# ETM-Code/eirgrid

Hardware: AMD Instinct MI355X
Metric: 26-year episodes/sec (higher is better)
Workload: dtype f64

## Files before the change

### eirgrid_amd/csrc/eg_api.cpp

```cpp
#include <algorithm>
#include <cstdlib>
#include <cstring>

#include "eg_device_tables.h"
#include "eg_host.h"
#include "eg_policy_internal.h"

namespace eg {
namespace {
thread_local std::string g_error;
}
void set_error(const std::string& s) { g_error = s; }
}

using namespace eg;

void eg_host_tables::index() {
  auto F = [&](const char* n, const std::vector<double>& v) { f64[n] = {v.data(), (int64_t)v.size()}; };
  auto I = [&](const char* n, const std::vector<int32_t>& v) { i32[n] = {v.data(), (int64_t)v.size()}; };
  F("usage", H.usage); F("population", H.population); F("pre_co2", H.pre_co2); F("pre_tg", H.pre_tg); F("pre_ig", H.pre_ig);
  F("pre_sg", H.pre_sg); F("pre_optot", H.pre_optot); F("te", H.te); F("coastf", H.coastf); F("dr", H.dr); F("m03", H.m03);
  F("t12", H.t12); F("cc", H.cc); F("out_mw", H.out_mw); F("co2_t", H.co2_t); F("offv", H.offv); F("offc", H.offc);
  F("inflation", H.inflation); F("carbon_price", H.carbon_price);
  f64["size_factor"] = {&H.size_factor, 1};
  I("pre_opcnt", H.pre_opcnt); I("cls", H.cls); I("rclass", H.rclass); I("marine", H.marine); I("reach", H.reach);
  I("existing_online", H.existing_online);
}

namespace {
struct Options {
  bool helper_off = false, helper_all = false;
  bool heavy_slots_auto = true; uint32_t heavy_slots_wanted = 4096;
  uint32_t heavy_slots_max = 0;
  bool side_stream_plain = false;
  bool replay_hoist = false;
  int coop_force = 0;
  bool solo_on = true;
  uint32_t solo_tiles = 1u;
};
Options read_options() {
  Options o;
  if (const char* hv = std::getenv("EIRGRID_HELPER_WAVES")) { o.helper_off = std::string(hv) == "0"; o.helper_all = std::string(hv) == "all"; }
  if (const char* hs = std::getenv("EIRGRID_HEAVY_SLOTS")) { o.heavy_slots_wanted = (uint32_t)std::strtoul(hs, nullptr, 10); o.heavy_slots_auto = false; }
  o.heavy_slots_max = uint32_t((size_t(64) << 30) / (size_t(kRadiusClasses) * 2624 * sizeof(double)));
  if (const char* hg = std::getenv("EIRGRID_HEAVY_POOL_GB"))
    o.heavy_slots_max = uint32_t(std::min(double((1u << 20) - 1u), std::max(0.0, std::atof(hg)) * double(size_t(1) << 30) / double(size_t(kRadiusClasses) * 2624 * sizeof(double))));
  if (o.heavy_slots_max > (1u << 20) - 1u) o.heavy_slots_max = (1u << 20) - 1u;
  if (o.heavy_slots_wanted > o.heavy_slots_max) o.heavy_slots_wanted = o.heavy_slots_max;
  if (const char* sp = std::getenv("EIRGRID_SIDE_STREAM")) o.side_stream_plain = std::string(sp) == "plain";
  if (const char* rh = std::getenv("EIRGRID_REPLAY_HOIST")) o.replay_hoist = rh[0] == '1';
  if (const char* cf = std::getenv("EIRGRID_COOP_FORCE")) o.coop_force = std::atoi(cf);
  if (const char* so = std::getenv("EIRGRID_REPLAY_SOLO")) o.solo_on = so[0] != '0';
  if (const char* st = std::getenv("EIRGRID_SOLO_TILES")) o.solo_tiles = st[0] != '0' ? 1u : 0u;
  return o;
}

int collect_timing(eg_ctx* c, int count = -1) {
  if (count < 0 || count > c->ring_pending) count = c->ring_pending;
  for (; count > 0; --count) {
    const int i = (c->ring_head - c->ring_pending + 2 * eg_ctx::kTimingRing) % eg_ctx::kTimingRing;
    const bool heavy = c->ev_used[i] & 1, lean = c->ev_used[i] & 2;
    float best = 0.f, sum = 0.f;
    for (int a = 0; a < 2; ++a)
      for (int b = 0; b < 2; ++b) {
        if (!(a ? lean : heavy) || !(b ? lean : heavy)) continue;
        EG_HIP(hipEventSynchronize(c->ev[i][2 * b + 1]));
        float ms = 0.f;
        EG_HIP(hipEventElapsedTime(&ms, c->ev[i][2 * a], c->ev[i][2 * b + 1]));
        if (a == b) sum += ms;
        if (ms > best) best = ms;
      }
    c->total_ms += double(best); c->grids_ms += double(sum); c->n_launches += 1; c->ring_pending -= 1;
  }
  return EG_OK;
}
}
static bool env_starts(const char* name, char ch) { const char* e = std::getenv(name); return e && e[0] == ch; }
bool eg::stats_replicas_off() { static const bool off = env_starts("EIRGRID_STATS_REPLICAS", '0'); return off; }
bool eg::fetch_full() { static const bool full = env_starts("EIRGRID_FETCH_FULL", '1'); return full; }

int eg::ensure_outputs(eg_ctx* c, uint32_t n) {
  const size_t bytes = size_t(n) * rec::stride + size_t(n) * sizeof(double);
  if (bytes <= c->d_out.count) return EG_OK;
  c->out = DevOut{};
  EG_HIP(c->d_out.reserve(bytes));
  c->out.base = c->d_out;
// ... 198 lines not shown
  return EG_OK;
}

extern "C" {

const char* eg_last_error(void) { return g_error.c_str(); }

int32_t eg_device_count(void) {
  int n = 0;
  if (hipGetDeviceCount(&n) != hipSuccess) return 0;
  return n;
}

eg_ctx* eg_create(int32_t device_ordinal, const eg_world* world) {
  if (!world || world->n_settlements < 0 || world->n_existing < 0 || world->n_coast < 0) { set_error("eg_create: bad world"); return nullptr; }
  int n = 0;
  if (hipGetDeviceCount(&n) != hipSuccess || n <= 0) { set_error("eg_create: no HIP device (this library has no CPU path)"); return nullptr; }
  if (device_ordinal < 0 || device_ordinal >= n) { set_error("eg_create: device ordinal out of range"); return nullptr; }
  if (hipSetDevice(device_ordinal) != hipSuccess) { set_error("eg_create: hipSetDevice failed"); return nullptr; }
  int cus = 0;
  if (hipDeviceGetAttribute(&cus, hipDeviceAttributeMultiprocessorCount, device_ordinal) != hipSuccess) cus = 0;
  const Options opt = read_options();
  eg_ctx* c = new eg_ctx();
  c->device = device_ordinal;
  c->helper_max_episodes = opt.helper_off ? 0u : opt.helper_all ? 0xFFFFFFFFu : 4u * (uint32_t)(cus > 0 ? cus : 0);
  c->heavy_slots_wanted = opt.heavy_slots_wanted; c->heavy_slots_auto = opt.heavy_slots_auto; c->heavy_slots_max = opt.heavy_slots_max;
  build_tables(*world, c->tables.H);
  c->tables.index();
  std::vector<uint8_t> blob;
  BlobInfo info;
  int rc = build_device_blob(c->tables.H, blob, info);
  if (rc == EG_OK) {
    c->dev.n_variants = info.n_variants; c->dev.size_factor = c->tables.H.size_factor; c->dev.n_existing = world->n_existing;
    c->dev.solo_tiles = opt.solo_tiles;
    if (!info.box_list_fits) c->heavy_slots_wanted = 0;
    c->hoist_supported = info.hoist_supported; c->hoist_on = info.hoist_supported && opt.replay_hoist;
    c->coop_force = opt.coop_force; c->solo_on = opt.solo_on;
    rc = create_device_state(c, blob, opt.side_stream_plain);
  }
  if (rc != EG_OK) { eg_destroy(c); return nullptr; }
  return c;
}

void eg_destroy(eg_ctx* c) {
  if (!c) return;
  (void)hipSetDevice(c->device);
  (void)hipDeviceSynchronize();
  for (int i = 0; i < eg_ctx::kTimingRing; ++i)
    for (int k = 0; k < 4; ++k) if (c->ev[i][k]) (void)hipEventDestroy(c->ev[i][k]);
  if (c->stream_heavy) (void)hipStreamDestroy(c->stream_heavy);
  for (int i = 0; i < eg_ctx::kTimingRing; ++i) { if (c->ev_fork[i]) (void)hipEventDestroy(c->ev_fork[i]); if (c->ev_go[i]) (void)hipEventDestroy(c->ev_go[i]); if (c->ev_join[i]) (void)hipEventDestroy(c->ev_join[i]); }
  delete c;
}

eg_host_tables* eg_host_tables_create(const eg_world* world) {
  if (!world || world->n_settlements < 0 || world->n_existing < 0 || world->n_coast < 0) { set_error("eg_host_tables_create: bad world"); return nullptr; }
  eg_host_tables* h = new eg_host_tables();
  build_tables(*world, h->H);
  h->index();
  return h;
}
void eg_host_tables_free(eg_host_tables* h) { delete h; }
int32_t eg_host_tables_f64(const eg_host_tables* h, const char* name, const double** ptr, int64_t* len) {
  return h ? find_table("eg_host_tables_f64", h->f64, name, ptr, len) : EG_ERR_BAD_ARG;
}
int32_t eg_host_tables_i32(const eg_host_tables* h, const char* name, const int32_t** ptr, int64_t* len) {
  return h ? find_table("eg_host_tables_i32", h->i32, name, ptr, len) : EG_ERR_BAD_ARG;
// ... 240 lines not shown
```

### eirgrid_amd/csrc/eg_internal.h

```cpp
#pragma once
#include <cstddef>
#include <cstdint>
#include <string>
#include <vector>

#include "eirgrid_hip.h"

namespace eg {

constexpr int kYears = EG_YEARS;
constexpr int kTypes = EG_N_TYPES;
constexpr int kCells = EG_CELLS;
constexpr int kGrid = EG_GRID;
constexpr int kRadiusClasses = 6;
constexpr int kMaxReach = 12;
constexpr int kMults = 3;
constexpr int kOffsetTypes = 4;
constexpr int kPsStride = 2624;
constexpr int kDrCompact = 352;
constexpr int kLdsGens = EG_ONCHIP_GENS;
constexpr int kShortReplayMax = 96;
constexpr int kMaxVariants = 12;
constexpr int kTileW = 8;
constexpr int kTileCols = (kGrid + kTileW - 1) / kTileW;
// ... 60 lines not shown
constexpr size_t m03 = a16(dr + 8 * kRadiusClasses * 169);
constexpr size_t t12 = a16(m03 + 8 * kCells);
constexpr size_t offv = a16(t12 + 8 * kYears * kTypes);
constexpr size_t offc = a16(offv + 8 * kYears * kOffsetTypes * kYears);
constexpr size_t cc = a16(offc + 8 * kYears * kOffsetTypes * kMults);
constexpr size_t ps = a16(cc + 8 * size_t(kYears) * kTypes * kYears * kMults * 2);
constexpr size_t hv_box = a16(ps + sizeof(PsRec) * size_t(kYears) * kMaxVariants * kPsStride);
constexpr size_t dr_meta = a16(hv_box + 4 * (1024 + 16));
constexpr size_t dr_compact = a16(dr_meta + 4 * 16);
constexpr size_t pbase = a16(dr_compact + 8 * size_t(kDrCompact));
constexpr size_t pcell = a16(pbase + 8 * size_t(kYears) * kMaxVariants * kPcStride);
constexpr size_t hv_lists = a16(pcell + 4 * size_t(kYears) * kMaxVariants * kPcStride);
constexpr size_t hv_quads = a16(hv_lists + 4 * size_t(64) * 1024);
constexpr size_t te_cell = a16(hv_quads + 4 * 64);
constexpr size_t coastf = a16(te_cell + 8 * size_t(kYears) * kRadiusClasses * kCells);
constexpr size_t cbase = a16(coastf + 8 * size_t(kCells));
constexpr size_t crank = a16(cbase + 8 * size_t(kYears) * kMaxVariants * kCells);
constexpr size_t ucell = a16(crank + 2 * size_t(kYears) * kMaxVariants * kCells);
constexpr size_t umax = a16(ucell + 8 * size_t(kMaxVariants) * kCells);
constexpr size_t rmax = a16(umax + 8 * size_t(kMaxVariants) * 64);
constexpr size_t total = a16(rmax + 8 * size_t(kYears) * kMaxVariants * 64);
}

struct DevTables {
  const uint8_t* base;
  double size_factor;
  int32_t n_existing;
  int32_t n_variants;
  uint32_t heavy_slots, heavy_epoch;
  uint8_t* heavy;
  unsigned* heavy_claim;
  double* heavy_tiles;
  uint32_t solo_tiles;
#define EG_TAB(name, type) EG_HD const type* name() const { return reinterpret_cast<const type*>(base + tab::name); }
  EG_TAB(usage, double) EG_TAB(population, double)
  EG_TAB(pre_co2, double) EG_TAB(pre_tg, double) EG_TAB(pre_ig, double) EG_TAB(pre_sg, double) EG_TAB(pre_optot, double)
  EG_TAB(inflation, double) EG_TAB(carbon_price, double) EG_TAB(out_mw, double) EG_TAB(co2_t, double)
  EG_TAB(pre_opcnt, int32_t) EG_TAB(variant, int32_t) EG_TAB(cls, int32_t) EG_TAB(rclass, int32_t) EG_TAB(marine, int32_t)
  EG_TAB(reach, int32_t)
  EG_TAB(dr, double) EG_TAB(m03, double) EG_TAB(t12, double) EG_TAB(offv, double) EG_TAB(offc, double) EG_TAB(cc, double)
  EG_TAB(ps, PsRec) EG_TAB(pbase, double) EG_TAB(pcell, uint32_t) EG_TAB(hv_lists, uint32_t) EG_TAB(hv_quads, int32_t) EG_TAB(dr_meta, int32_t) EG_TAB(dr_compact, double)
  EG_TAB(te_cell, double) EG_TAB(coastf, double) EG_TAB(cbase, double) EG_TAB(crank, uint16_t) EG_TAB(ucell, double) EG_TAB(umax, double) EG_TAB(rmax, double)
#undef EG_TAB
};

struct DevState {
  double learning_rate, exploration_rate;
  double best_metrics[4];
  double rel_improvement, immediate_weight;
  double p_best_score, p_threshold, p_adaptive_lr, p_stagnation;
  double boost_others, boost_noop, eps_main, scaled_power;
  uint32_t stall, iteration_count;
  int32_t has_best, has_cw, noop_boost, has_lists, p_forced;
  uint32_t heur_min, heur_max;
  uint32_t n_improvements;
  int32_t improved_last;
  uint32_t failed_total;
};
static_assert(sizeof(DevState) % 8 == 0, "state layout");
struct DevImprovement { double score, metrics[4]; uint32_t iteration, pad; };

namespace snap {
constexpr size_t kBestCap = 4096;
constexpr int kPolRow = 128, kPolTotMain = 61, kPolTotDeficit = 62, kPolTotCount = 63, kPolDw = 64, kPolScaledTotal = 79, kPolCw = 80;
constexpr int kPolYear = 101;
constexpr size_t pol = 0;
// ... 263 lines not shown
```

### eirgrid_amd/csrc/eg_replay_solo.h

```cpp
#pragma once

namespace solo {

struct Lists {
  unsigned long long gen_pack;
  __device__ __forceinline__ static int* words() { return reinterpret_cast<int*>(sm.pol); }
  __device__ __forceinline__ int gpack_at(int i) const {
    __builtin_amdgcn_fence(__ATOMIC_RELEASE, "workgroup");
    return tail_u16(gen_pack, i);
  }
  __device__ __forceinline__ void gpack_put(int, int) const {}
  __device__ __forceinline__ void opack_put(int, int) const {}
  __device__ __forceinline__ int cls(int t) const { return (sm.type_info[t] >> 12) & 3; }
  __device__ __forceinline__ double out(int t) const { return sm.type_out[t]; }
  __device__ __forceinline__ void year_end(int yi, int ngen, int noff) const { words()[yi] = ngen; words()[EG_YEARS + yi] = noff; }
  __device__ __forceinline__ void finish(int run_pos, int def_pos, int act_pos, int ngen, int noff, unsigned long long bytes) const {
    int* w = words();
    w[52] = run_pos; w[53] = def_pos; w[54] = act_pos; w[55] = ngen; w[56] = noff;
    *reinterpret_cast<unsigned long long*>(w + 58) = bytes;
  }
};
static_assert(snap::kPolRow * 8 >= 60 * 4, "the script's lengths fit the policy row block");

constexpr int kEnt = 8;
struct Entries { int base[kEnt], delta[kEnt], dd[kEnt]; double fac[kEnt]; };
__device__ __forceinline__ void load_entries(Entries& E, int lane) {
#pragma unroll
  for (int k = 0; k < kEnt; ++k) {
    const uint32_t en = sh2.box[k * kWave + lane];
    const int rc = (int)(en >> 19), di = (int)(en & 31u) - 16, dj = (int)((en >> 5) & 31u) - 16;
    E.base[k] = rc * kFieldStride; E.delta[k] = di * kGrid + dj; E.dd[k] = (di & 0xFFFF) | (int)((unsigned)dj << 16);
    E.fac[k] = factor_by_q<false>(rc, (int)offsetof(Smem, dr), (int)((en >> 10) & 511u));
  }
}
template <int kN>
__device__ __forceinline__ void field_add(unsigned long long field_addr, const Entries& E, int cell) {
  const GlobalF64 base = (GlobalF64)field_addr;
  const int gi = cell / kGrid, gj = cell - gi * kGrid;
  double val[kN]; int off[kN];
#pragma unroll
  for (int k = 0; k < kN; ++k) {
    const int ci = gi + (int)(short)(E.dd[k] & 0xFFFF), cj = gj + (E.dd[k] >> 16);
    const bool inside = (unsigned)ci < (unsigned)kGrid && (unsigned)cj < (unsigned)kGrid;
    off[k] = E.base[k] + (inside ? cell + E.delta[k] : kCells);
    val[k] = field_load(base + off[k]);
  }
#pragma unroll
  for (int k = 0; k < kN; ++k) base[off[k]] = val[k] * E.fac[k];
}

}

__global__ void __launch_bounds__(kWave, EG_HEAVY_WAVES) k_replay_solo(DevTables T, DevSnapshot S_in, DevOut O, unsigned long long first_index, uint32_t n_episodes,
                                                                       const uint8_t* __restrict__ replay_mask, uint32_t replay_period, long long* stats,
                                                                       EpisodeMap emap) {
  const int lane = threadIdx.x;
  if (blockIdx.x >= emap.count) return;
  if (S_in.plan_pool == nullptr && !(S_in.state()->has_lists && S_in.resident_list_len() > kShortReplayMax)) return;
  if (emap.hoist_seq != 0ull && *emap.hoist == emap.hoist_seq) return;
  const uint32_t e = map_episode(emap, blockIdx.x);
  if (e >= n_episodes) return;
  DevSnapshot S = S_in;
  load_state(S);
  plan_lists(S, e);
  const bool replay = replay_mask != nullptr ? replay_mask[e] != 0 : (replay_period != 0u && S.has_best_actions && (first_index + e) % replay_period == 0ull);
  if (!replay || !S.has_best_actions) return;
#ifdef EG_SOLO_STAMPS
  unsigned long long cs[8] = {0, 0, 0, 0, 0, 0, 0, 0}, cs_last = __builtin_readcyclecounter();
#define EG_SS(slot) do { const unsigned long long now_ = __builtin_readcyclecounter(); cs[slot] += now_ - cs_last; cs_last = now_; } while (0)
#else
#define EG_SS(slot) do {} while (0)
#endif
  load_static_tables(T, lane, true);
#if defined(EG_SOLO_STAMPS) && defined(EG_STAMPS)
  if (lane < 8) sm.hdbg[lane >> 2][lane & 3] = 0ull;
#endif
  wave_sync();
  EG_SS(0);

  solo::Lists ls{(unsigned long long)O.gen_pack(e)};
  if (!rs::script(T, S, O, e, ls, lane)) return;
  __builtin_amdgcn_fence(__ATOMIC_RELEASE, "workgroup");
  wave_sync();
  EG_SS(1);
  const int* words = solo::Lists::words();
  const int n_gens = __builtin_amdgcn_readfirstlane(words[55]);

  Episode ep;
  ep.ngen = 0; ep.chunks = 0; ep.heavy = -1; ep.heavy_classes = 0; ep.heavy_quads = 0;
  uint16_t* gen_cell = O.gen_cell(e);
  const ListTail tail = {(unsigned long long)gen_cell, (unsigned long long)O.gen_pack(e), (unsigned long long)O.off_pack(e)};
  PrefixCache prefix_cache0 = {0.0, -1, 0};
  uint32_t search_seq = 0;
  int tile_variants = 0;
  int pk_block = 0;
  solo::Entries E;
#pragma unroll
  for (int k = 0; k < solo::kEnt; ++k) { E.base[k] = 0; E.delta[k] = 0; E.dd[k] = 0; E.fac[k] = 1.0; }
  for (int g = 0; g < n_gens; ++g) {
    if ((g & (kWave - 1)) == 0) pk_block = g + lane < n_gens ? tail_u16(tail.gen_pack, g + lane) : 0;
    const int pk = __builtin_amdgcn_readlane(pk_block, g & (kWave - 1));
    const int t = pk & 15, yi = (pk >> 4) & 31, m = pk >> 9;
    double m03v = 0.0;
    int cell = -1;
    bool placed = false;
    auto between = [] {};
    EG_SS(2);
    if (ep.ngen >= kHeavyGens && ep.heavy != -2) {
      const unsigned long long slot_bytes = (unsigned long long)(kRadiusClasses * kFieldStride) * 8ull;
      if (ep.heavy == -1) ep.heavy = heavy_claim(T, lane);
      if (ep.heavy >= 0) {
        const int info = __builtin_amdgcn_readfirstlane(sm.type_info[t]);
        const int hv = info & 15, hrc = (info >> 4) & 15;
        const unsigned long long class_addr = (unsigned long long)T.heavy + (unsigned long long)ep.heavy * slot_bytes + (unsigned long long)(hrc * kFieldStride) * 8ull;
        const unsigned long long tiles_addr = (unsigned long long)T.heavy_tiles + (unsigned long long)((ep.heavy * kMaxVariants + hv) * 64) * 8ull;
        if (!((ep.heavy_classes >> hrc) & 1)) {
          heavy_build_class<false>(class_addr, tail.gen_cell, lane, hrc, throughput_table(info), (info >> 8) & 15, ep.ngen);
          ep.heavy_classes |= 1 << hrc;
          ep.heavy_quads = __builtin_amdgcn_readfirstlane(T.hv_quads()[ep.heavy_classes]);
          wave_sync();
#pragma unroll
          for (int k = 0; k < kBoxLds / kWave; ++k) sh2.box[k * kWave + lane] = T.hv_lists()[ep.heavy_classes * 1024 + k * kWave + lane];
          wave_sync();
          solo::load_entries(E, lane);
        }
        int hr = kTilesUndecided;
        if (T.solo_tiles && !((tile_variants >> hv) & 1)) {
          ((GlobalF64)tiles_addr)[lane] = T.umax()[hv * 64 + lane];
          tile_variants |= 1 << hv;
        }
        if (T.solo_tiles) hr = place_tiles((unsigned long long)T.base, yi * kMaxVariants + hv, class_addr, tiles_addr, tail.gen_cell, T.size_factor, lane, hrc, throughput_table(info), ep.ngen);
        if (hr == kTilesUndecided) {
          const size_t yv = (size_t)(yi * kMaxVariants + hv) * kPsStride, yc = (size_t)(yi * kMaxVariants + hv) * kPcStride;
          hr = place_heavy<false>((unsigned long long)(T.ps() + yv), (unsigned long long)(T.pbase() + yc), (unsigned long long)(T.pcell() + yc), class_addr,
                                  tail.gen_cell, T.size_factor, lane, hrc, throughput_table(info), ep.ngen);
        }
        if (hr >= 0) { cell = hr & 0xFFFF; ep.chunks += hr >> 16; placed = true; }
      }
    }
    if (!placed && ep.ngen > kLdsGens) {
      const int info = __builtin_amdgcn_readfirstlane(sm.type_info[t]);
      const int xr = place_exact_long<false>((unsigned long long)(T.ps() + (size_t)(yi * kMaxVariants + (info & 15)) * kPsStride), tail.gen_cell,
                                             T.size_factor, lane, (info >> 4) & 15, throughput_table(info), ep.ngen);
      cell = xr < 0 ? -1 : (xr & 0xFFFF);
      if (xr >= 0) ep.chunks += xr >> 16;
      placed = true;
    }
    if (!placed) cell = __builtin_amdgcn_readfirstlane(place_search<0>(T, lane, yi, t, ep.ngen, nullptr, &m03v, prefix_cache0, between, ep.chunks, &search_seq));
    EG_SS(3);
    if (cell >= 0 && ep.heavy_classes != 0) {
      const unsigned long long field_addr = (unsigned long long)T.heavy + (unsigned long long)ep.heavy * ((unsigned long long)(kRadiusClasses * kFieldStride) * 8ull);
      ep.chunks += 2 * ep.heavy_quads;
      const unsigned long long hv_list = (unsigned long long)(T.hv_lists() + ep.heavy_classes * 1024);
      if (ep.heavy_quads == 1) solo::field_add<4>(field_addr, E, cell);
      else solo::field_add<8>(field_addr, E, cell);
      if (ep.heavy_quads == 3) heavy_add_body<false, 4>(field_addr, hv_list, lane, cell, 8);
      else if (ep.heavy_quads >= 4) heavy_add_body<false, 8>(field_addr, hv_list, lane, cell, 8);
    }
    if (cell < 0) {
      if (lane == 0 && ep.heavy >= 0) emap.solo[blockIdx.x] = (emap.solo_seq << 21) | (1ull << 20) | (unsigned long long)ep.heavy;
      return;
    }
    if (lane == 0) {
      if (ep.ngen < kLdsGens) { sm.gcell[ep.ngen] = (uint16_t)(cell | (t << 12)); sm.gbm[ep.ngen] = (uint8_t)(yi | (m << 5)); }
      gen_cell[ep.ngen] = (uint16_t)cell;
    }
    wave_sync();
    ep.ngen += 1;
    EG_SS(4);
  }

  __builtin_amdgcn_fence(__ATOMIC_RELEASE, "workgroup");
  wave_sync();
  double total_cost = 0.0, total_credit = 0.0, total_sales = 0.0;
  double last[7] = {0.0, 0.0, 0.0, 0.0, 0.0, 0.0, 0.0};
  for (int y0 = 0; y0 < kYears; y0 += 4) {
    const rs::YearRow q = rs::books_quad(T, S_in, O, e, y0, words, words + EG_YEARS, lane, [](const uint16_t* list, int i) { return tail_u16((unsigned long long)list, i); });
#pragma unroll
    for (int r = 0; r < 4; ++r) {
      const int yi = y0 + r;
      if (yi >= kYears) break;
#pragma unroll
      for (int k = 0; k < 7; ++k) last[k] = readlane_f64(q.v[k], 16 * r);
      total_cost = yi == 0 ? last[0] : total_cost + last[0];
      total_credit = yi == 0 ? last[1] : total_credit + last[1];
      total_sales = yi == 0 ? last[2] : total_sales + last[2];
      if (S_in.write_yearly && lane == 0) {
        double* row = O.yearly(e) + yi * EG_YEARLY_FIELDS;
        row[EG_Y_TOTAL_COST] = total_cost; row[EG_Y_TOTAL_CREDIT] = total_credit; row[EG_Y_TOTAL_SALES] = total_sales;
      }
    }
  }
  EG_SS(5);
  if (lane == 0) {
    O.metrics(e)[0] = last[3]; O.metrics(e)[1] = last[4]; O.metrics(e)[2] = last[5];
    O.metrics(e)[3] = last[6] >= 0.0 ? 1.0 : 0.0;
    *O.status(e) = EG_EP_OK; *O.n_gens(e) = words[55]; *O.n_offsets(e) = words[56];
    *O.n_draws(e) = 0ull;
    *O.bytes_moved(e) = (double)*reinterpret_cast<const unsigned long long*>(words + 58);
    *O.n_chunks(e) = (uint32_t)ep.chunks;
  }
  if (stats != nullptr) {
    __builtin_amdgcn_fence(__ATOMIC_RELEASE, "workgroup");
    __builtin_amdgcn_fence(__ATOMIC_ACQUIRE, "workgroup");
    wave_sync();
    StatsParams P;
    load_stats_params(S, P);
    episode_update_stats(O, S, P, e, lane, stats, 1ull, emap.stats_rep ? (int)(blockIdx.x % (uint32_t)kStatsReplicas) : -1);
  }
  EG_SS(6);
#ifdef EG_SOLO_STAMPS
  if (lane == 0) {
    unsigned long long* dbg = (unsigned long long*)(O.act_log(e) + EG_ACT_CAP - 256);
    for (int i = 0; i < 8; ++i) dbg[i] = cs[i];
#ifdef EG_STAMPS
    for (int i = 0; i < 3; ++i) { dbg[8 + i] = sm.hdbg[0][i]; dbg[11 + i] = sm.hdbg[1][i]; }
    dbg[14] = sm.hdbg[1][3];
#endif
  }
#endif
  if (lane == 0) emap.solo[blockIdx.x] = emap.solo_seq;
}
```

### eirgrid_amd/csrc/eg_rollout.hip

```cpp
#include <hip/hip_runtime.h>
#include <cstddef>
#include <hip/hip_ext.h>

#include "eg_internal.h"

#define EG_DETPOW_QUAL __device__ __forceinline__
#include "eg_detpow.h"
#define EG_RM __device__ __forceinline__
#include "eg_reduced_math.h"

namespace eg {
namespace {

constexpr int kWave = 64;
constexpr int kD2Max = 144, kD2Stride = 146;
constexpr int kCmdYear = 1 << 30;
constexpr int kHelperWaves = 1;
constexpr int kSpinCap = 1 << 20;
constexpr int kSearchLost = -2;
constexpr double kMinWeight = 0.0001;
constexpr double kMaxWeight = 0.999;
constexpr double kMaxCost = 50000000000.0;
constexpr int kBattery = 12, kPeaker = 8;
constexpr int kNothing = 60, kFirstOffset = 45, kFirstOther = 57;
// ... 1031 lines not shown
  int ncand = 0, solo = -1;
  if (__ballot(l2 >= thr) == 0ull) {
    const unsigned long long m1 = __ballot(lm >= thr);
    ncand = __popcll(m1);
    if (ncand == 1) solo = __ffsll((long long)m1) - 1;
    if ((m1 >> lane) & 1ull) sm.gstage[1][__popcll(m1 & ((1ull << lane) - 1ull))] = (__double2loint(lm) & 63) * kWave + lane;
  } else {
    for (int k = 0; k < K; ++k) {
      const double approx = pb_at(k * kWave + lane) * field_at(pc_at(k * kWave + lane));
      const unsigned long long m = __ballot(approx >= thr && approx > 0.0);
      if (m != 0ull) {
        const int pos = ncand + __popcll(m & ((1ull << lane) - 1ull));
        if (((m >> lane) & 1ull) && pos < kWave) sm.gstage[1][pos] = k * kWave + lane;
        ncand += __popcll(m);
      }
    }
  }
  if (ncand > kWave || ncand == 0) return kSearchFallback;
  wave_sync();
#ifdef EG_STAMPS
  asm volatile("s_waitcnt vmcnt(0)" ::: "memory");
  const unsigned long long ts2 = __builtin_readcyclecounter();
#endif
  const ChunkBest b = heavy_exact<kLatency>(list_addr, tail_cells, size_factor, lane, rc, tbl, ngen_s, ncand, ncand == 1 && solo >= 0 ? __builtin_amdgcn_readlane(lcell, solo) : -1);
  if (!(b.score > 0.0)) return kSearchFallback;
#ifdef EG_STAMPS
  if (lane == 0) { sm.hdbg[0][0] += ts1 - ts0; sm.hdbg[0][1] += ts2 - ts1; sm.hdbg[0][2] += __builtin_readcyclecounter() - ts2; sm.hdbg[1][0] += (unsigned long long)K; sm.hdbg[1][1] += (unsigned long long)ncand; sm.hdbg[1][2] += 1ull; }
#endif
  return heavy_result(b, lane, K, ncand);
}

constexpr int kTilesUndecided = -4;
static_assert(kTileW * kTileW == kWave, "a cell of a tile per lane");
__device__ __noinline__ int place_tiles(unsigned long long tab_addr, int yv, unsigned long long class_addr, unsigned long long tiles_addr,
                                        unsigned long long tail_cells, double size_factor, int lane, int rc, int tbl, int ngen) {
#ifdef EG_STAMPS
  const unsigned long long ts0 = __builtin_readcyclecounter();
#endif
  asm volatile("s_waitcnt vmcnt(0)" ::: "memory");
  const int ngen_s = __builtin_amdgcn_readfirstlane(ngen);
  constexpr int kChunks = (kCells + kWave - 1) / kWave, kGroup = 4, kGroups = (kChunks + kGroup - 1) / kGroup;
  constexpr double kKeep = 1.0 - 0x1p-30, kKeepTile = 1.0 - 0x1p-29;
  constexpr int kNoTile = 63;
  static_assert(kNoTile >= kTiles && (kNoTile / kTileCols) * kTileW >= kGrid, "kNoTile is off the grid");
  auto uniform_u64 = [](unsigned long long a) { return ((unsigned long long)(unsigned)__builtin_amdgcn_readfirstlane((int)(a >> 32)) << 32) | (unsigned)__builtin_amdgcn_readfirstlane((int)a); };
  const unsigned long long tab_s = uniform_u64(tab_addr), a_s = uniform_u64(class_addr), t_s = uniform_u64(tiles_addr);
  const unsigned long long yv_s = (unsigned long long)(unsigned)__builtin_amdgcn_readfirstlane(yv);
  const unsigned long long cb_s = tab_s + tab::cbase + yv_s * (8ull * kCells), rk_s = tab_s + tab::crank + yv_s * (2ull * kCells);
  const unsigned long long pb_s = tab_s + tab::pbase + yv_s * (8ull * kPcStride), rm_s = tab_s + tab::rmax + yv_s * (8ull * 64);
  const unsigned long long uc_s = tab_s + tab::ucell + (yv_s % kMaxVariants) * (8ull * kCells);
  const GlobalF64 gmax = (GlobalF64)t_s;
  auto field_at = [&](int cell) { return __hip_atomic_load((GlobalF64)(a_s + (unsigned long long)((unsigned)cell * 8u)), __ATOMIC_RELAXED, __HIP_MEMORY_SCOPE_AGENT); };
  auto cb_at = [&](int cell) { return *(GlobalF64c)(cb_s + (unsigned long long)((unsigned)cell * 8u)); };
  auto uc_at = [&](int cell) { return *(GlobalF64c)(uc_s + (unsigned long long)((unsigned)cell * 8u)); };
  auto rk_at = [&](int cell) { return (int)*(const uint16_t __attribute__((address_space(1)))*)(rk_s + (unsigned long long)((unsigned)cell * 2u)); };
  const double gb = lane >= 1 && lane < kGroups ? *(GlobalF64c)(pb_s + (unsigned long long)((unsigned)(lane * kGroup * kWave) * 8u)) : 0.0;
  const double bound = lane < kTiles ? *(GlobalF64c)(rm_s + (unsigned long long)((unsigned)lane * 8u)) * field_load(gmax + lane) : 0.0;
  unsigned long long left = __ballot(bound > 0.0);
  if (left == 0ull) return kSearchFallback;
  const unsigned hb = (unsigned)__double2hiint(bound);
  const unsigned h1 = wave_max_u32(hb);
  int ta = __ffsll((long long)(left & __ballot(hb == h1))) - 1, tb = kNoTile;
  {
    const unsigned long long rest = left & ~(1ull << ta);
    const unsigned h2 = wave_max_u32(lane == ta ? 0u : hb);
    const unsigned long long second = rest & __ballot(hb == h2);
    if (rest != 0ull) tb = __ffsll((long long)(second != 0ull ? second : rest)) - 1;
  }
  double lm = 0.0, l2 = 0.0;
  int lrank = 0, lcell = -1;
#ifdef EG_STAMPS
  int tiles = 0;
#endif
  auto fold = [&](double v, int r, int c) {
    const double key = __hiloint2double(__double2hiint(v), (__double2loint(v) & ~63) | (r >> 6));
    const bool larger = key > lm;
    l2 = vmax64(l2, vmin64(lm, key));
    lm = vmax64(lm, key);
    lrank = larger ? r : lrank; lcell = larger ? c : lcell;
  };
#pragma nounroll
  for (;;) {
    left &= ~(1ull << ta) & ~(1ull << tb);
    const int ia = (ta / kTileCols) * kTileW + (lane >> 3), ja = (ta % kTileCols) * kTileW + (lane & 7);
    const int ib = (tb / kTileCols) * kTileW + (lane >> 3), jb = (tb % kTileCols) * kTileW + (lane & 7);
    const bool ina = ia < kGrid && ja < kGrid, inb = ib < kGrid && jb < kGrid;
    const int ca = ina ? ia * kGrid + ja : 0, cb = inb ? ib * kGrid + jb : 0;
    const double fa = field_at(ca), fb = field_at(cb), pa = cb_at(ca), pb = cb_at(cb), ua = uc_at(ca), ub = uc_at(cb);
    const int ra = rk_at(ca), rb = rk_at(cb);
    fold(ina ? pa * fa : 0.0, ra, ca);
    fold(inb ? pb * fb : 0.0, rb, cb);
    const unsigned gha = wave_max_u32(ina ? (unsigned)__double2hiint(ua * fa) : 0u), ghb = wave_max_u32(inb ? (unsigned)__double2hiint(ub * fb) : 0u);
    if (lane == 0) {
      gmax[ta] = __hiloint2double((int)gha, -1);
      if (tb < kTiles) gmax[tb] = __hiloint2double((int)ghb, -1);
    }
#ifdef EG_STAMPS
    tiles += tb < kTiles ? 2 : 1;
#endif
    const double m_lo = __hiloint2double((int)wave_max_u32((unsigned)__double2hiint(lm)), 0);
    left &= __ballot(bound >= m_lo * kKeepTile);
    if (left == 0ull) break;
    ta = __ffsll((long long)left) - 1;
    const unsigned long long rest = left & (left - 1ull);
    tb = rest != 0ull ? __ffsll((long long)rest) - 1 : kNoTile;
  }
  const double M = wave_max_f64(lm);
  if (!(M >= 1e-250)) return kSearchFallback;
#ifdef EG_STAMPS
  const unsigned long long ts1 = __builtin_readcyclecounter();
#endif
  const double thr = M * kKeep;
  if (__ballot(l2 >= thr) != 0ull) return kTilesUndecided;
  const int gstar = (__double2loint(M) & 63) / kGroup;
  const double m_hi = __hiloint2double(__double2hiint(M), 0);
  const unsigned long long stops = __ballot(lane > gstar && lane < kGroups && !(gb >= m_hi * kKeep));
  const int g_stop = stops != 0ull ? __ffsll((long long)stops) - 1 : kGroups;
  const int K = kGroup * g_stop < kChunks ? kGroup * g_stop : kChunks;
  const unsigned long long m1 = __ballot(lm >= thr && lrank < K * kWave);
  const int ncand = __popcll(m1);
  if (ncand == 0) return kTilesUndecided;
  if (ncand > 1) {
// ... 1335 lines not shown
    double* s_sw = s_scratch + (tid >> 6) * 64; double* s_ss = s_scratch + 16 * 64 + (tid >> 6) * 64;
    for (int y = tid >> 6; y < Y; y += 16) stalled_tables_year(snap_base, y, tid & 63, st.stall, s_sw, s_ss);
  }
#ifdef EG_STAMPS
  __syncthreads();
  if (tid == 0) {
    const unsigned long long t_end = wall_clock64();
    zero_stats[4] = (long long)(dbg_t[2] - dbg_t[0]);
    zero_stats[5] = (long long)(dbg_t[4] - dbg_t[2]);
    zero_stats[6] = (long long)(dbg_t[5] - dbg_t[4]);
    zero_stats[7] = (long long)(t_end - dbg_t[5]);
  }
#endif
}

#endif
}

int launch_rollout_throughput(int kind, const DevTables& t, const DevSnapshot& s, const DevOut& o, uint64_t seed, uint64_t first_index, uint32_t n,
                              const uint8_t* d_replay_mask, uint32_t replay_period, long long* d_stats, uint32_t count, uint32_t mode,
                              const uint32_t* index, uint32_t off, uint32_t period, const unsigned long long* hoist, unsigned long long hoist_seq,
                              uint32_t stats_rep, uint32_t same_index, unsigned long long* solo, unsigned long long solo_seq, void* stream, void* ev0, void* ev1);
#ifdef EG_TU_THROUGHPUT
int launch_rollout_throughput(int kind, const DevTables& t, const DevSnapshot& s, const DevOut& o, uint64_t seed, uint64_t first_index, uint32_t n,
                              const uint8_t* d_replay_mask, uint32_t replay_period, long long* d_stats, uint32_t count, uint32_t mode,
                              const uint32_t* index, uint32_t off, uint32_t period, const unsigned long long* hoist, unsigned long long hoist_seq,
                              uint32_t stats_rep, uint32_t same_index, unsigned long long* solo, unsigned long long solo_seq, void* stream, void* ev0, void* ev1) {
  EpisodeMap map{};
  map.count = count; map.mode = mode; map.index = index; map.off = off; map.period = period; map.hoist = hoist; map.hoist_seq = hoist_seq; map.stats_rep = stats_rep; map.same_index = same_index;
  map.solo = solo; map.solo_seq = solo_seq;
#define EG_LAUNCH_TP(kKind) hipExtLaunchKernelGGL((k_rollout<0, kKind>), dim3(map.count), dim3(kWave), 0, (hipStream_t)stream, (hipEvent_t)ev0, (hipEvent_t)ev1, 0, \
                                                  t, s, o, (unsigned long long)seed, (unsigned long long)first_index, n, d_replay_mask, replay_period, d_stats, map)
  if (kind == kReplayLong) {
    if (solo_seq != 0ull)
      hipLaunchKernelGGL(k_replay_solo, dim3(map.count), dim3(kWave), 0, (hipStream_t)stream, t, s, o, (unsigned long long)first_index, n, d_replay_mask, replay_period,
                         d_stats, map);
    EG_LAUNCH_TP(kReplayLong);
  }
  else if (kind == kReplayShort) EG_LAUNCH_TP(kReplayShort);
  else EG_LAUNCH_TP(kLean);
#undef EG_LAUNCH_TP
  return (int)hipGetLastError();
}
#else
namespace {
template <int kKind>
void launch_variant(bool helper_waves, const DevTables& t, const DevSnapshot& s, const DevOut& o, uint64_t seed, uint64_t first_index, uint32_t n,
                    const uint8_t* d_replay_mask, uint32_t replay_period, long long* d_stats, const EpisodeMap& map, void* stream, void* ev0, void* ev1) {
  if (helper_waves)
    hipExtLaunchKernelGGL((k_rollout<kHelperWaves, kKind>), dim3(map.count), dim3(kWave * (1 + kHelperWaves)), 0, (hipStream_t)stream,
                          (hipEvent_t)ev0, (hipEvent_t)ev1, 0, t, s, o, (unsigned long long)seed, (unsigned long long)first_index, n,
                          d_replay_mask, replay_period, d_stats, map);
  else
    (void)launch_rollout_throughput(kKind, t, s, o, seed, first_index, n, d_replay_mask, replay_period, d_stats, map.count, map.mode, map.index, map.off, map.period,
                                    map.hoist, map.hoist_seq, map.stats_rep, map.same_index, map.solo, map.solo_seq, stream, ev0, ev1);
}
}

int launch_rollout(const DevTables& t, const DevSnapshot& s, const DevOut& o, uint64_t seed, uint64_t first_index,
                   uint32_t n, const uint8_t* d_replay_mask, uint32_t replay_period, long long* d_stats_packet, const RolloutPlan& p) {
  if (n == 0) return 0;
  const bool rep = d_stats_packet != nullptr && p.d_stats_rep != nullptr;
  long long* d_stats = rep ? p.d_stats_rep : d_stats_packet;
  if (p.plans) {
    EpisodeMap ms{}, ml{};
    ms.count = p.n_short; ms.mode = 1u; ms.index = p.d_index;
    ml.count = p.n_heavy - p.n_short; ml.mode = 1u; ml.index = p.d_index_long;
// ... 262 lines not shown
```

Baseline: 8.702 million.

## Lazily build heavy class fields per tile in solo replay

```diff
diff --git a/eirgrid_amd/csrc/eg_api.cpp b/eirgrid_amd/csrc/eg_api.cpp
--- a/eirgrid_amd/csrc/eg_api.cpp
+++ b/eirgrid_amd/csrc/eg_api.cpp
@@ -37,6 +37,7 @@
   int coop_force = 0;
   bool solo_on = true;
   uint32_t solo_tiles = 1u;
+  uint32_t solo_lazy = 384u;
 };
 Options read_options() {
   Options o;
@@ -52,6 +53,7 @@
   if (const char* cf = std::getenv("EIRGRID_COOP_FORCE")) o.coop_force = std::atoi(cf);
   if (const char* so = std::getenv("EIRGRID_REPLAY_SOLO")) o.solo_on = so[0] != '0';
   if (const char* st = std::getenv("EIRGRID_SOLO_TILES")) o.solo_tiles = st[0] != '0' ? 1u : 0u;
+  if (const char* sl = std::getenv("EIRGRID_SOLO_LAZY")) o.solo_lazy = std::string(sl) == "all" ? 0xFFFFFFFFu : (uint32_t)std::strtoul(sl, nullptr, 10);
   return o;
 }
 
@@ -316,7 +318,7 @@
   int rc = build_device_blob(c->tables.H, blob, info);
   if (rc == EG_OK) {
     c->dev.n_variants = info.n_variants; c->dev.size_factor = c->tables.H.size_factor; c->dev.n_existing = world->n_existing;
-    c->dev.solo_tiles = opt.solo_tiles;
+    c->dev.solo_tiles = opt.solo_tiles; c->dev.solo_lazy = opt.solo_lazy;
     if (!info.box_list_fits) c->heavy_slots_wanted = 0;
     c->hoist_supported = info.hoist_supported; c->hoist_on = info.hoist_supported && opt.replay_hoist;
     c->coop_force = opt.coop_force; c->solo_on = opt.solo_on;
diff --git a/eirgrid_amd/csrc/eg_internal.h b/eirgrid_amd/csrc/eg_internal.h
--- a/eirgrid_amd/csrc/eg_internal.h
+++ b/eirgrid_amd/csrc/eg_internal.h
@@ -116,6 +116,7 @@
   unsigned* heavy_claim;
   double* heavy_tiles;
   uint32_t solo_tiles;
+  uint32_t solo_lazy;
 #define EG_TAB(name, type) EG_HD const type* name() const { return reinterpret_cast<const type*>(base + tab::name); }
   EG_TAB(usage, double) EG_TAB(population, double)
   EG_TAB(pre_co2, double) EG_TAB(pre_tg, double) EG_TAB(pre_ig, double) EG_TAB(pre_sg, double) EG_TAB(pre_optot, double)
diff --git a/eirgrid_amd/csrc/eg_replay_solo.h b/eirgrid_amd/csrc/eg_replay_solo.h
--- a/eirgrid_amd/csrc/eg_replay_solo.h
+++ b/eirgrid_amd/csrc/eg_replay_solo.h
@@ -51,9 +51,10 @@
 
 }
 
-__global__ void __launch_bounds__(kWave, EG_HEAVY_WAVES) k_replay_solo(DevTables T, DevSnapshot S_in, DevOut O, unsigned long long first_index, uint32_t n_episodes,
-                                                                       const uint8_t* __restrict__ replay_mask, uint32_t replay_period, long long* stats,
-                                                                       EpisodeMap emap) {
+template <bool kLazy>
+__device__ __forceinline__ void replay_solo_episode(const DevTables& T, const DevSnapshot& S_in, const DevOut& O, unsigned long long first_index, uint32_t n_episodes,
+                                                    const uint8_t* __restrict__ replay_mask, uint32_t replay_period, long long* stats,
+                                                    const EpisodeMap& emap) {
   const int lane = threadIdx.x;
   if (blockIdx.x >= emap.count) return;
   if (S_in.plan_pool == nullptr && !(S_in.state()->has_lists && S_in.resident_list_len() > kShortReplayMax)) return;
@@ -93,6 +94,7 @@
   PrefixCache prefix_cache0 = {0.0, -1, 0};
   uint32_t search_seq = 0;
   int tile_variants = 0;
+  const bool lazy = kLazy && T.solo_tiles != 0u && (uint32_t)n_gens <= T.solo_lazy;
   int pk_block = 0;
   solo::Entries E;
 #pragma unroll
@@ -115,22 +117,32 @@
         const unsigned long long class_addr = (unsigned long long)T.heavy + (unsigned long long)ep.heavy * slot_bytes + (unsigned long long)(hrc * kFieldStride) * 8ull;
         const unsigned long long tiles_addr = (unsigned long long)T.heavy_tiles + (unsigned long long)((ep.heavy * kMaxVariants + hv) * 64) * 8ull;
         if (!((ep.heavy_classes >> hrc) & 1)) {
-          heavy_build_class<false>(class_addr, tail.gen_cell, lane, hrc, throughput_table(info), (info >> 8) & 15, ep.ngen);
+          if (lazy) { if (lane < kTiles) ((GlobalU16)(class_addr + 8ull * kTileCounters))[lane] = (unsigned short)0; }
+          else heavy_build_class<false>(class_addr, tail.gen_cell, lane, hrc, throughput_table(info), (info >> 8) & 15, ep.ngen);
           ep.heavy_classes |= 1 << hrc;
           ep.heavy_quads = __builtin_amdgcn_readfirstlane(T.hv_quads()[ep.heavy_classes]);
-          wave_sync();
-#pragma unroll
-          for (int k = 0; k < kBoxLds / kWave; ++k) sh2.box[k * kWave + lane] = T.hv_lists()[ep.heavy_classes * 1024 + k * kWave + lane];
-          wave_sync();
-          solo::load_entries(E, lane);
+          if (!lazy) {
+            wave_sync();
+#pragma unroll
+            for (int k = 0; k < kBoxLds / kWave; ++k) sh2.box[k * kWave + lane] = T.hv_lists()[ep.heavy_classes * 1024 + k * kWave + lane];
+            wave_sync();
+            solo::load_entries(E, lane);
+          }
         }
         int hr = kTilesUndecided;
         if (T.solo_tiles && !((tile_variants >> hv) & 1)) {
           ((GlobalF64)tiles_addr)[lane] = T.umax()[hv * 64 + lane];
           tile_variants |= 1 << hv;
         }
-        if (T.solo_tiles) hr = place_tiles((unsigned long long)T.base, yi * kMaxVariants + hv, class_addr, tiles_addr, tail.gen_cell, T.size_factor, lane, hrc, throughput_table(info), ep.ngen);
+        if (lazy) hr = place_tiles<true>((unsigned long long)T.base, yi * kMaxVariants + hv, class_addr, tiles_addr, tail.gen_cell, T.size_factor, lane, hrc | (((info >> 8) & 15) << 8), throughput_table(info), ep.ngen);
+        else if (T.solo_tiles) hr = place_tiles<false>((unsigned long long)T.base, yi * kMaxVariants + hv, class_addr, tiles_addr, tail.gen_cell, T.size_factor, lane, hrc, throughput_table(info), ep.ngen);
         if (hr == kTilesUndecided) {
+          if (lazy) {
+            tiles_catch_up_all(class_addr, tail.gen_cell, lane, hrc, throughput_table(info), (info >> 8) & 15, ep.ngen);
+#if defined(EG_SOLO_STAMPS) && defined(EG_STAMPS)
+            if (lane == 0) sm.hdbg[0][3] += 1ull << 40;
+#endif
+          }
           const size_t yv = (size_t)(yi * kMaxVariants + hv) * kPsStride, yc = (size_t)(yi * kMaxVariants + hv) * kPcStride;
           hr = place_heavy<false>((unsigned long long)(T.ps() + yv), (unsigned long long)(T.pbase() + yc), (unsigned long long)(T.pcell() + yc), class_addr,
                                   tail.gen_cell, T.size_factor, lane, hrc, throughput_table(info), ep.ngen);
@@ -152,10 +164,12 @@
       const unsigned long long field_addr = (unsigned long long)T.heavy + (unsigned long long)ep.heavy * ((unsigned long long)(kRadiusClasses * kFieldStride) * 8ull);
       ep.chunks += 2 * ep.heavy_quads;
       const unsigned long long hv_list = (unsigned long long)(T.hv_lists() + ep.heavy_classes * 1024);
-      if (ep.heavy_quads == 1) solo::field_add<4>(field_addr, E, cell);
-      else solo::field_add<8>(field_addr, E, cell);
-      if (ep.heavy_quads == 3) heavy_add_body<false, 4>(field_addr, hv_list, lane, cell, 8);
-      else if (ep.heavy_quads >= 4) heavy_add_body<false, 8>(field_addr, hv_list, lane, cell, 8);
+      if (!lazy) {
+        if (ep.heavy_quads == 1) solo::field_add<4>(field_addr, E, cell);
+        else solo::field_add<8>(field_addr, E, cell);
+        if (ep.heavy_quads == 3) heavy_add_body<false, 4>(field_addr, hv_list, lane, cell, 8);
+        else if (ep.heavy_quads >= 4) heavy_add_body<false, 8>(field_addr, hv_list, lane, cell, 8);
+      }
     }
     if (cell < 0) {
       if (lane == 0 && ep.heavy >= 0) emap.solo[blockIdx.x] = (emap.solo_seq << 21) | (1ull << 20) | (unsigned long long)ep.heavy;
@@ -216,8 +230,20 @@
 #ifdef EG_STAMPS
     for (int i = 0; i < 3; ++i) { dbg[8 + i] = sm.hdbg[0][i]; dbg[11 + i] = sm.hdbg[1][i]; }
     dbg[14] = sm.hdbg[1][3];
+    dbg[15] = sm.hdbg[0][3];
 #endif
   }
 #endif
   if (lane == 0) emap.solo[blockIdx.x] = emap.solo_seq;
 }
+
+__global__ void __launch_bounds__(kWave, EG_HEAVY_WAVES) k_replay_solo(DevTables T, DevSnapshot S_in, DevOut O, unsigned long long first_index, uint32_t n_episodes,
+                                                                       const uint8_t* __restrict__ replay_mask, uint32_t replay_period, long long* stats,
+                                                                       EpisodeMap emap) {
+  replay_solo_episode<false>(T, S_in, O, first_index, n_episodes, replay_mask, replay_period, stats, emap);
+}
+__global__ void __launch_bounds__(kWave, EG_HEAVY_WAVES) k_replay_lazy(DevTables T, DevSnapshot S_in, DevOut O, unsigned long long first_index, uint32_t n_episodes,
+                                                                       const uint8_t* __restrict__ replay_mask, uint32_t replay_period, long long* stats,
+                                                                       EpisodeMap emap) {
+  replay_solo_episode<true>(T, S_in, O, first_index, n_episodes, replay_mask, replay_period, stats, emap);
+}
diff --git a/eirgrid_amd/csrc/eg_rollout.hip b/eirgrid_amd/csrc/eg_rollout.hip
--- a/eirgrid_amd/csrc/eg_rollout.hip
+++ b/eirgrid_amd/csrc/eg_rollout.hip
@@ -1087,8 +1087,69 @@
 
 constexpr int kTilesUndecided = -4;
 static_assert(kTileW * kTileW == kWave, "a cell of a tile per lane");
+constexpr int kNoTile = 63;
+static_assert(kNoTile >= kTiles && (kNoTile / kTileCols) * kTileW >= kGrid, "kNoTile is off the grid");
+
+constexpr int kTileCounters = kCells + 1;
+static_assert((kFieldStride - kTileCounters) * 8 >= kTiles * 2 && EG_MAX_GENS <= 0xFFFF, "a 16-bit counter per tile fits behind a class's cells");
+__device__ __forceinline__ int tiles_refresh(unsigned long long a_s, int applied, int ta, int tb, int lane, int rc, int tbl, int reach, int ngen_s,
+                                             unsigned long long tail_cells, double& fa, double& fb) {
+  const int cap = factor_cap<false>(tbl);
+  const int ra = (ta / kTileCols) * kTileW, ca = (ta % kTileCols) * kTileW, rb = (tb / kTileCols) * kTileW, cb = (tb % kTileCols) * kTileW;
+  const int ia = ra + (lane >> 3), ja = ca + (lane & 7), ib = rb + (lane >> 3), jb = cb + (lane & 7);
+  const int aa = __builtin_amdgcn_readlane(applied, ta), ab = tb < kTiles ? __builtin_amdgcn_readlane(applied, tb) : ngen_s;
+  fa = aa == 0 ? 1.0 : fa; fb = ab == 0 ? 1.0 : fb;
+  int folded = 0;
+  const unsigned span = (unsigned)(kTileW - 1 + 2 * reach);
+  for (int gb = (aa < ab ? aa : ab) & ~(kWave - 1); gb < ngen_s; gb += kWave) {
+    const int gc = list_cell(tail_cells, gb, lane, ngen_s, 0), g = gb + lane;
+    const int gi = gc / kGrid, gj = gc - gi * kGrid;
+    const bool na = g >= aa && g < ngen_s && (unsigned)(gi - ra + reach) <= span && (unsigned)(gj - ca + reach) <= span;
+    const bool nb = g >= ab && g < ngen_s && (unsigned)(gi - rb + reach) <= span && (unsigned)(gj - cb + reach) <= span;
+    const int gij = gi | (gj << 8);
+    unsigned long long near = __ballot(na || nb);
+    while (near != 0ull) {
+      const int j = __ffsll((long long)near) - 1;
+      const int w = __builtin_amdgcn_readlane(gij, j), si = w & 255, sj = w >> 8;
+      int qa = (ia - si) * (ia - si) + (ja - sj) * (ja - sj), qb = (ib - si) * (ib - si) + (jb - sj) * (jb - sj);
+      qa = qa < cap && gb + j >= aa ? qa : cap;
+      qb = qb < cap && gb + j >= ab ? qb : cap;
+      fa = fa * factor_by_q<false>(rc, tbl, qa);
+      fb = fb * factor_by_q<false>(rc, tbl, qb);
+      near &= near - 1ull;
+      ++folded;
+    }
+  }
+  if (ia < kGrid && ja < kGrid) *(GlobalF64)(a_s + (unsigned long long)((unsigned)(ia * kGrid + ja) * 8u)) = fa;
+  if (ib < kGrid && jb < kGrid) *(GlobalF64)(a_s + (unsigned long long)((unsigned)(ib * kGrid + jb) * 8u)) = fb;
+  if (lane == 0) {
+    const GlobalU16 cnt = (GlobalU16)(a_s + 8ull * kTileCounters);
+    cnt[ta] = (unsigned short)ngen_s;
+    if (tb < kTiles) cnt[tb] = (unsigned short)ngen_s;
+  }
+  return folded;
+}
+__device__ __noinline__ void tiles_catch_up_all(unsigned long long class_addr, unsigned long long tail_cells, int lane, int rc, int tbl, int reach, int ngen) {
+  asm volatile("s_waitcnt vmcnt(0)" ::: "memory");
+  const int ngen_s = __builtin_amdgcn_readfirstlane(ngen);
+  const unsigned long long a_s = ((unsigned long long)(unsigned)__builtin_amdgcn_readfirstlane((int)(class_addr >> 32)) << 32) | (unsigned)__builtin_amdgcn_readfirstlane((int)class_addr);
+  const int applied = lane < kTiles ? tail_u16(a_s + 8ull * kTileCounters, lane) : 0;
+  if (__ballot(lane < kTiles && applied != ngen_s) == 0ull) return;
+#pragma nounroll
+  for (int ta = 0; ta < kTiles; ta += 2) {
+    const int tb = ta + 1 < kTiles ? ta + 1 : kNoTile;
+    const int ia = (ta / kTileCols) * kTileW + (lane >> 3), ja = (ta % kTileCols) * kTileW + (lane & 7);
+    const int ib = (tb / kTileCols) * kTileW + (lane >> 3), jb = (tb % kTileCols) * kTileW + (lane & 7);
+    const int ca = ia < kGrid && ja < kGrid ? ia * kGrid + ja : 0, cb = ib < kGrid && jb < kGrid ? ib * kGrid + jb : 0;
+    double fa = field_load((GlobalF64)a_s + ca), fb = field_load((GlobalF64)a_s + cb);
+    tiles_refresh(a_s, applied, ta, tb, lane, rc, tbl, reach, ngen_s, tail_cells, fa, fb);
+  }
+}
+
+template <bool kLazy>
 __device__ __noinline__ int place_tiles(unsigned long long tab_addr, int yv, unsigned long long class_addr, unsigned long long tiles_addr,
-                                        unsigned long long tail_cells, double size_factor, int lane, int rc, int tbl, int ngen) {
+                                        unsigned long long tail_cells, double size_factor, int lane, int rc_in, int tbl, int ngen) {
+  const int rc = kLazy ? rc_in & 255 : rc_in, reach = kLazy ? rc_in >> 8 : 0;
 #ifdef EG_STAMPS
   const unsigned long long ts0 = __builtin_readcyclecounter();
 #endif
@@ -1096,8 +1157,6 @@
   const int ngen_s = __builtin_amdgcn_readfirstlane(ngen);
   constexpr int kChunks = (kCells + kWave - 1) / kWave, kGroup = 4, kGroups = (kChunks + kGroup - 1) / kGroup;
   constexpr double kKeep = 1.0 - 0x1p-30, kKeepTile = 1.0 - 0x1p-29;
-  constexpr int kNoTile = 63;
-  static_assert(kNoTile >= kTiles && (kNoTile / kTileCols) * kTileW >= kGrid, "kNoTile is off the grid");
   auto uniform_u64 = [](unsigned long long a) { return ((unsigned long long)(unsigned)__builtin_amdgcn_readfirstlane((int)(a >> 32)) << 32) | (unsigned)__builtin_amdgcn_readfirstlane((int)a); };
   const unsigned long long tab_s = uniform_u64(tab_addr), a_s = uniform_u64(class_addr), t_s = uniform_u64(tiles_addr);
   const unsigned long long yv_s = (unsigned long long)(unsigned)__builtin_amdgcn_readfirstlane(yv);
@@ -1111,6 +1170,8 @@
   auto rk_at = [&](int cell) { return (int)*(const uint16_t __attribute__((address_space(1)))*)(rk_s + (unsigned long long)((unsigned)cell * 2u)); };
   const double gb = lane >= 1 && lane < kGroups ? *(GlobalF64c)(pb_s + (unsigned long long)((unsigned)(lane * kGroup * kWave) * 8u)) : 0.0;
   const double bound = lane < kTiles ? *(GlobalF64c)(rm_s + (unsigned long long)((unsigned)lane * 8u)) * field_load(gmax + lane) : 0.0;
+  int applied = 0;
+  if constexpr (kLazy) applied = lane < kTiles ? tail_u16(a_s + 8ull * kTileCounters, lane) : 0;
   unsigned long long left = __ballot(bound > 0.0);
   if (left == 0ull) return kSearchFallback;
   const unsigned hb = (unsigned)__double2hiint(bound);
@@ -1141,8 +1202,17 @@
     const int ib = (tb / kTileCols) * kTileW + (lane >> 3), jb = (tb % kTileCols) * kTileW + (lane & 7);
     const bool ina = ia < kGrid && ja < kGrid, inb = ib < kGrid && jb < kGrid;
     const int ca = ina ? ia * kGrid + ja : 0, cb = inb ? ib * kGrid + jb : 0;
-    const double fa = field_at(ca), fb = field_at(cb), pa = cb_at(ca), pb = cb_at(cb), ua = uc_at(ca), ub = uc_at(cb);
+    double fa = field_at(ca), fb = field_at(cb);
+    const double pa = cb_at(ca), pb = cb_at(cb), ua = uc_at(ca), ub = uc_at(cb);
     const int ra = rk_at(ca), rb = rk_at(cb);
+    if constexpr (kLazy) {
+      const int folded = tiles_refresh(a_s, applied, ta, tb, lane, rc, tbl, reach, ngen_s, tail_cells, fa, fb);
+#ifdef EG_STAMPS
+      if (lane == 0) sm.hdbg[0][3] += (unsigned long long)folded;
+#else
+      (void)folded;
+#endif
+    }
     fold(ina ? pa * fa : 0.0, ra, ca);
     fold(inb ? pb * fb : 0.0, rb, cb);
     const unsigned gha = wave_max_u32(ina ? (unsigned)__double2hiint(ua * fa) : 0u), ghb = wave_max_u32(inb ? (unsigned)__double2hiint(ub * fb) : 0u);
@@ -2544,7 +2614,10 @@
 #define EG_LAUNCH_TP(kKind) hipExtLaunchKernelGGL((k_rollout<0, kKind>), dim3(map.count), dim3(kWave), 0, (hipStream_t)stream, (hipEvent_t)ev0, (hipEvent_t)ev1, 0, \
                                                   t, s, o, (unsigned long long)seed, (unsigned long long)first_index, n, d_replay_mask, replay_period, d_stats, map)
   if (kind == kReplayLong) {
-    if (solo_seq != 0ull)
+    if (solo_seq != 0ull && t.solo_tiles != 0u && t.solo_lazy != 0u)
+      hipLaunchKernelGGL(k_replay_lazy, dim3(map.count), dim3(kWave), 0, (hipStream_t)stream, t, s, o, (unsigned long long)first_index, n, d_replay_mask, replay_period,
+                         d_stats, map);
+    else if (solo_seq != 0ull)
       hipLaunchKernelGGL(k_replay_solo, dim3(map.count), dim3(kWave), 0, (hipStream_t)stream, t, s, o, (unsigned long long)first_index, n, d_replay_mask, replay_period,
                          d_stats, map);
     EG_LAUNCH_TP(kReplayLong);
```

After: 9.559 million (median of 6 runs). +9.8%, better.
